# someone-in-somewhere/multimodal_rag

Measured on AMD Instinct MI355X. Metric: chunks embedded/sec + queries/sec top_k=5 over 1M×768 at 1/2/4/8 GPUs, higher is better.
Workload: dtype f16

## Files before the change

multimodal_rag_amd/csrc/search.hip:

```cpp
#include "slab_ring.h"

#include <stdlib.h>

using namespace mmrag;

namespace mmrag_impl {

template <int DT, int WN, int K, int NSTAGE, int NW, bool SEEDED>
__global__ __launch_bounds__(64 * NW, NW / 4) void cosine_topk_kernel(const KParams p) {
#if defined(__HIP_DEVICE_COMPILE__)
#include "slab_ring_body.inc"
#endif
}

template <int K>
struct FullList {
    float v[K];
    long long r[K];
    __device__ inline void init() {
#pragma unroll
        for (int i = 0; i < K; ++i) {
            v[i] = NEG_INF;
            r[i] = LLONG_MAX;
        }
// ... 193 lines not shown
    else launch_main<DT, 8, 0, 2, 16>(p, grid, s);
}

int deep_filter_launch(int dtype, int WN, const KParams &p, int grid_x, int grid_y, hipStream_t s) {
    if (dtype == MMRAG_F8E4M3) return f8_filter_launch(WN, p, grid_x, grid_y, s);
    const dim3 grid(grid_x, grid_y);
    if (dtype == MMRAG_F32) launch_filter<MMRAG_F32>(WN, p, grid, s);
    else if (dtype == MMRAG_F16) launch_filter<MMRAG_F16>(WN, p, grid, s);
    else launch_filter<MMRAG_BF16>(WN, p, grid, s);
    MMRAG_CHECK_HIP(hipGetLastError());
    return MMRAG_OK;
}

template <typename RowT>
int launch_merge(int K, const float *cs, const RowT *cr, long long n_cand, long long inner,
                 long long outer_stride, long long q_stride, int B, int k_out, long long row_offset,
                 float *out_s, long long *out_r, hipStream_t s, float *thr0 = nullptr, float *seed_s = nullptr,
                 int *seed_r = nullptr, long long seed_q_stride = 0) {
    if (K == 5)
        merge_topk_kernel<5, RowT><<<B, 256, 0, s>>>(cs, cr, n_cand, inner, outer_stride, q_stride, k_out,
                                                     row_offset, out_s, out_r, thr0, seed_s, seed_r, seed_q_stride);
    else if (K == 10)
        merge_topk_kernel<10, RowT><<<B, 256, 0, s>>>(cs, cr, n_cand, inner, outer_stride, q_stride, k_out,
                                                      row_offset, out_s, out_r, thr0, seed_s, seed_r, seed_q_stride);
    else
        merge_topk_kernel<20, RowT><<<B, 256, 0, s>>>(cs, cr, n_cand, inner, outer_stride, q_stride, k_out,
                                                      row_offset, out_s, out_r, thr0, seed_s, seed_r, seed_q_stride);
    return MMRAG_OK;
}

__global__ void fill_empty_kernel(float *s, long long *r, long long total) {
    const long long i = (long long)blockIdx.x * blockDim.x + threadIdx.x;
    if (i < total) {
        s[i] = NEG_INF;
        r[i] = -1;
    }
}

__global__ void fill_seed_empty_kernel(float *s, int *r, long long q_stride, int K, long long n_queries) {
    const long long q = (long long)blockIdx.x * blockDim.x + threadIdx.x;
    if (q < n_queries)
        for (int i = 0; i < K; ++i) {
            s[q * q_stride + i] = NEG_INF;
            r[q * q_stride + i] = INT_MAX;
        }
}

}
using namespace mmrag_impl;

extern "C" {

struct WsLayout {
    size_t entries, off_r, off_thr, off_ts, off_tr, off_cnt, cnt_bytes, off_pub, off_pthr, off_tk, xch_end, total;
};
static WsLayout ws_layout(const Plan &pl) {
    WsLayout w;
    w.entries = (size_t)pl.b_pad * pl.n_lists * pl.K;
    w.off_r = w.entries * sizeof(float);
    w.off_thr = w.off_r + w.entries * sizeof(int);
    w.off_ts = w.off_thr + (size_t)pl.b_pad * sizeof(float);
    w.off_tr = (w.off_ts + (size_t)pl.b_pad * pl.K * sizeof(float) + 15) / 16 * 16;
    w.off_cnt = (w.off_tr + (size_t)pl.b_pad * pl.K * sizeof(long long) + 63) / 64 * 64;
    w.cnt_bytes = 0;
    w.off_pub = w.off_cnt + w.cnt_bytes;
    w.off_pthr = w.off_pub + (pl.qs_room ? (size_t)pl.b_pad * pl.grid_x * sizeof(float) : 0);
    w.off_tk = w.off_pthr + (pl.qs_room ? (size_t)pl.b_pad * sizeof(float) : 0);
    w.xch_end = w.off_tk + (pl.qs_room ? ((size_t)pl.grid_y * sizeof(unsigned) + 63) / 64 * 64 : 0);
    w.total = w.xch_end;
    return w;
}

size_t mmrag_cosine_topk_workspace_bytes(int B, int64_t n, int k) {
    if (B <= 0 || n < 0 || k < 1 || k > MMRAG_MAX_K) return 0;
    return ws_layout(make_plan(B, n, k)).total + 256;
}

static int check_search_args(const void *q, const void *corpus, int B, int64_t n, int d, int64_t ld, int dtype,
                             int k) {
    MMRAG_CHECK_ARG(dtype >= 0 && dtype <= MMRAG_F8E4M3, "cosine_topk: bad dtype %d", dtype);
    MMRAG_CHECK_ARG(B > 0, "cosine_topk: B must be positive (got %d)", B);
    MMRAG_CHECK_ARG(k >= 1 && k <= MMRAG_MAX_K, "cosine_topk: k=%d outside 1..%d", k, MMRAG_MAX_K);
    MMRAG_CHECK_ARG(n >= 0 && n < (int64_t)INT_MAX - TM, "cosine_topk: n=%lld out of range", (long long)n);
    MMRAG_CHECK_ARG(d > 0 && ld >= d, "cosine_topk: need 0 < d <= ld (d=%d ld=%lld)", d, (long long)ld);
    const int64_t row_bytes = ld * esize(dtype);
    MMRAG_CHECK_ARG(row_bytes % SLAB == 0,
                    "cosine_topk: row bytes %lld not a multiple of %d (use mmrag_padded_dim)", (long long)row_bytes, SLAB);
    MMRAG_CHECK_ARG(row_bytes * TM < (int64_t)UINT_MAX, "cosine_topk: rows too long");
    MMRAG_CHECK_ARG(q, "cosine_topk: null q");
    MMRAG_CHECK_ARG(n == 0 || corpus, "cosine_topk: null corpus");
    MMRAG_CHECK_ARG(((uintptr_t)q % 16) == 0 && ((uintptr_t)corpus % 16) == 0,
                    "cosine_topk: q/corpus must be 16-byte aligned");
    return MMRAG_OK;
}

int mmrag_internal_cosine_topk_lists_ex(const void *q, const void *corpus, int B, int64_t n, int d, int64_t ld,
                                        int dtype, int k, const uint32_t *alive_bits, void *workspace,
                                        size_t workspace_bytes, void *stream, unsigned dbg) {
    if (int st = check_search_args(q, corpus, B, n, d, ld, dtype, k)) return st;
    if (n == 0) return MMRAG_OK;
    const Plan pl = make_plan(B, n, k, dbg);
    const WsLayout wl = ws_layout(pl);
    if (!workspace || workspace_bytes < wl.total) {
        set_error("cosine_topk: workspace %zu bytes < required %zu", workspace_bytes, wl.total);
        return MMRAG_EWORKSPACE;
    }
    MMRAG_CHECK_ARG(((uintptr_t)workspace % 16) == 0, "cosine_topk: workspace must be 16-byte aligned");

    KParams p;
    p.q = (const char *)q;
    p.corpus = (const char *)corpus;
    p.alive_bits = alive_bits;
    p.cand_s = (float *)workspace;
    p.cand_r = (int *)((char *)workspace + wl.off_r);
    p.n = n;
    p.B = B;
    p.row_bytes = (unsigned)(ld * esize(dtype));
    p.n_tiles = pl.n_tiles;
    p.n_lists = pl.n_lists;
    p.tile0 = 0;
    p.thr0 = nullptr;
    p.dbg = dbg;
    p.stamps = ((dbg & DBG_QS_CLOCK) && workspace_bytes >= wl.total + 256 * (size_t)(pl.grid_x * pl.grid_y)) ? (unsigned long long *)((char *)workspace + wl.total) : nullptr;
    p.walkers = pl.grid_x;
    p.share_l2 = pl.grid_y > 1;
    p.sample_best = nullptr;
    p.pub_best = nullptr;
    p.pub_thr = nullptr;
    p.tickets = nullptr;
    p.p_static = INT_MAX / 2;
    hipStream_t s = (hipStream_t)stream;
    const size_t seed_off = (size_t)(pl.n_lists - 1) * pl.K;
    const int walk_mfma = (dbg & DBG_MFMA32) ? 32 : ((dbg & DBG_MFMA16) ? 16 : (pl.K == 5 ? QSW_DEFAULT_MFMA : 32));
    if (pl.qs_ok && !(dbg & DBG_OLD_QS) && qsw_supported(dtype, p.row_bytes, pl.K, walk_mfma)) {
        const int tiles = (int)((n + QS_TILE_ROWS - 1) / QS_TILE_ROWS);
        const int per = tiles / pl.grid_x;
        p.n_tiles = tiles;
        p.pub_best = nullptr;
        p.pub_thr = nullptr;
        p.tickets = nullptr;
        p.p_static = INT_MAX / 2;
        const bool seed = per >= 12 && !(dbg & DBG_NO_SEED);
        const bool dyn = pl.grid_y == 1 && per >= 24 && !(dbg & DBG_NO_DYN);
        if (seed || dyn) {
            MMRAG_CHECK_HIP(hipMemsetD32Async((hipDeviceptr_t)((char *)workspace + wl.off_pub), (int)TICKET0,
                                              (wl.xch_end - wl.off_pub) / 4, s));
            if (seed) {
                p.pub_best = (float *)((char *)workspace + wl.off_pub);
                p.pub_thr = (float *)((char *)workspace + wl.off_pthr);
            }
            if (dyn) {
                p.tickets = (unsigned *)((char *)workspace + wl.off_tk);
                const int tail = per / 10 > 3 ? per / 10 : 3;
                p.p_static = per - tail;
            }
        }
        if (int st = qsw_launch(dtype, pl.K, walk_mfma, p, pl.grid_x, pl.grid_y, s)) return st;
        MMRAG_CHECK_HIP(hipGetLastError());
        return MMRAG_OK;
    }
    if (pl.qs_ok && qs_supported(dtype, p.row_bytes, pl.K)) {
        const int tiles = (int)((n + QS_TILE_ROWS - 1) / QS_TILE_ROWS);
        float *thr0 = nullptr;
        if (pl.pre_tiles > 0) {
            KParams ks = p;
            ks.n_tiles = pl.pre_tiles * (TM / QS_TILE_ROWS);
            ks.sample_best = (float *)((char *)workspace + wl.off_pub);
            if (int st = qs_launch(dtype, pl.K, ks, pl.grid_x, pl.grid_y, s)) return st;
            thr0 = (float *)((char *)workspace + wl.off_thr);
            if (int st = qs_seed_thresholds(pl.K, ks.sample_best, pl.grid_x, pl.b_pad, thr0, s)) return st;
        }
        p.n_tiles = tiles;
        p.thr0 = thr0;
        if (int st = qs_launch(dtype, pl.K, p, pl.grid_x, pl.grid_y, s)) return st;
        MMRAG_CHECK_HIP(hipGetLastError());
        return MMRAG_OK;
    }
    auto run = [&](int tile0, int n_tiles, int grid_x, const float *thr0) -> int {
        KParams kp = p;
        kp.tile0 = tile0;
        kp.n_tiles = n_tiles;
        kp.thr0 = thr0;
        Plan lp = pl;
        lp.grid_x = grid_x;
        if (dtype == MMRAG_F8E4M3) return f8_lists_launch(lp.K, lp.WN, kp, lp.grid_x, lp.grid_y, s);
        if (dtype == MMRAG_F32) return dispatch_main<MMRAG_F32>(lp, kp, s);
        if (dtype == MMRAG_F16) return dispatch_main<MMRAG_F16>(lp, kp, s);
        return dispatch_main<MMRAG_BF16>(lp, kp, s);
    };
    if (pl.pre_tiles > 0) {
        float *thr0 = (float *)((char *)workspace + wl.off_thr);
        float *top_s = (float *)((char *)workspace + wl.off_ts);
        long long *top_r = (long long *)((char *)workspace + wl.off_tr);
        const int pre = pl.pre_tiles;
        const int pre_grid = pre < pl.grid_x ? pre : pl.grid_x;
        if (int st = run(0, pre, pre_grid, nullptr)) return st;
        MMRAG_CHECK_HIP(hipGetLastError());
        const long long n_cand = (long long)pre_grid * pl.K;
        launch_merge<int>(pl.K, p.cand_s, p.cand_r, n_cand, n_cand, 0, (long long)pl.n_lists * pl.K, B, pl.K, 0, top_s,
                          top_r, s, thr0, p.cand_s + seed_off, p.cand_r + seed_off, (long long)pl.n_lists * pl.K);
        MMRAG_CHECK_HIP(hipGetLastError());
        if (int st = run(pre, pl.n_tiles - pre, pl.grid_x, thr0)) return st;
    } else {
// ... 73 lines not shown
```

multimodal_rag_amd/csrc/search_qsw.hip:

```cpp
#include "search_shared.h"

#include <type_traits>
#include <utility>

using namespace mmrag;

namespace mmrag_impl {

namespace {

template <int DT>
struct WFrag;
template <>
struct WFrag<MMRAG_F16> {
    using T = half8_t;
};
template <>
struct WFrag<MMRAG_BF16> {
    using T = bf16x8_t;
};

template <typename F, int... I>
__device__ __forceinline__ void static_for_impl(F &&f, std::integer_sequence<int, I...>) {
    (f(std::integral_constant<int, I>{}), ...);
}
template <int N, typename F>
__device__ __forceinline__ void static_for(F &&f) {
    static_for_impl(f, std::make_integer_sequence<int, N>{});
}

constexpr int QSW_XCH = 2048 + 64;
constexpr int qsw_lists_bytes(int K, int MS) { return K * (MS == 32 ? 2 : 4) * QS_QROWS * 8; }

struct WRing {
    int G;
    int NST;
};
constexpr WRing qsw_ring(int NK, int K, int MS) {
#if defined(MMRAG_QSW_RING16)
    if (MS == 16 && NK % (MMRAG_QSW_RING16 / 10) == 0) return WRing{MMRAG_QSW_RING16 / 10, MMRAG_QSW_RING16 % 10};
#endif
    const int budget = 160 * 1024 - qsw_lists_bytes(K, MS) - QSW_XCH;
    for (int need = 4; need >= 3; --need)
        for (int g = 4; g >= 1; --g) {
            if (NK % g) continue;
            int nst = budget / (g * QS_TILE_ROWS * SLAB);
            if (nst > 6) nst = 6;
            if (nst >= need) return WRing{g, nst};
        }
    return WRing{1, 2};
}

#define MMRAG_QSW_S32(MNEMONIC, QC, C00, C01, C10, C11, ACC)                                                  \
    asm volatile("v_xad_u32 %[t], %[lo], %[xc], %[st]\n\t"                                                    \
                 "ds_read_b128 %[n0], %[t] offset:%[o0]\n\t"                                                  \
                 "ds_read_b128 %[n1], %[t] offset:%[o1]\n\t" MNEMONIC " %[c00], %[a0], %[q0], " C00 "\n\t"    \
                 MNEMONIC " %[c01], %[a0], %[q1], " C01 "\n\t" MNEMONIC " %[c10], %[a1], %[q0], " C10 "\n\t"  \
                 MNEMONIC " %[c11], %[a1], %[q1], " C11 "\n\t"                                                \
                 "s_waitcnt lgkmcnt(0)"                                                                       \
                 : [c00] ACC(c00), [c01] ACC(c01), [c10] ACC(c10), [c11] ACC(c11), [n0] "=&v"(n0),            \
                   [n1] "=&v"(n1), [t] "=&v"(tmp)                                                             \
                 : [a0] "v"(a0), [a1] "v"(a1), [q0] QC(q0), [q1] QC(q1), [lo] "v"(lo), [st] "s"(st),          \
                   [xc] "i"(XC), [o0] "i"(OFF0), [o1] "i"(OFF1))

template <int DT, bool QA, bool FIRST, int XC, int OFF0, int OFF1, typename FT>
__device__ __forceinline__ void qsw_stmt32(f32x16_t &c00, f32x16_t &c01, f32x16_t &c10, f32x16_t &c11, const FT a0,
                                           const FT a1, const FT q0, const FT q1, FT &n0, FT &n1, const unsigned lo,
                                           const unsigned st) {
    unsigned tmp;
    if constexpr (FIRST) {
        static_assert(QA, "the first k-step's Q fragments live in the accumulator file");
        if constexpr (DT == MMRAG_F16) MMRAG_QSW_S32("v_mfma_f32_32x32x16_f16", "a", "0", "0", "0", "0", "=&v");
        else MMRAG_QSW_S32("v_mfma_f32_32x32x16_bf16", "a", "0", "0", "0", "0", "=&v");
    } else if constexpr (DT == MMRAG_F16) {
        if constexpr (QA) MMRAG_QSW_S32("v_mfma_f32_32x32x16_f16", "a", "%[c00]", "%[c01]", "%[c10]", "%[c11]", "+v");
        else MMRAG_QSW_S32("v_mfma_f32_32x32x16_f16", "v", "%[c00]", "%[c01]", "%[c10]", "%[c11]", "+v");
    } else {
        if constexpr (QA) MMRAG_QSW_S32("v_mfma_f32_32x32x16_bf16", "a", "%[c00]", "%[c01]", "%[c10]", "%[c11]", "+v");
        else MMRAG_QSW_S32("v_mfma_f32_32x32x16_bf16", "v", "%[c00]", "%[c01]", "%[c10]", "%[c11]", "+v");
    }
}

#define MMRAG_QSW_S16(MNEMONIC, QC, D0, D1, D2, D3, D4, D5, D6, D7, ACC)                                      \
    asm volatile(MNEMONIC " %[d0], %[a0], %[q0], " D0 "\n\t"                                                  \
                 "ds_read_b128 %[n0], %[ad] offset:%[o0]\n\t" MNEMONIC " %[d1], %[a0], %[q1], " D1 "\n\t"     \
                 "ds_read_b128 %[n1], %[ad] offset:%[o1]\n\t" MNEMONIC " %[d2], %[a0], %[q2], " D2 "\n\t"     \
                 MNEMONIC " %[d3], %[a0], %[q3], " D3 "\n\t" MNEMONIC " %[d4], %[a1], %[q0], " D4 "\n\t"      \
                 MNEMONIC " %[d5], %[a1], %[q1], " D5 "\n\t" MNEMONIC " %[d6], %[a1], %[q2], " D6 "\n\t"      \
                 MNEMONIC " %[d7], %[a1], %[q3], " D7 "\n\t"                                                  \
                 "s_waitcnt lgkmcnt(0)"                                                                       \
                 : [d0] ACC(d0), [d1] ACC(d1), [d2] ACC(d2), [d3] ACC(d3), [d4] ACC(d4), [d5] ACC(d5),        \
                   [d6] ACC(d6), [d7] ACC(d7), [n0] "=&v"(n0), [n1] "=&v"(n1)                                 \
                 : [a0] "v"(a0), [a1] "v"(a1), [q0] QC(q0), [q1] QC(q1), [q2] QC(q2), [q3] QC(q3),            \
                   [ad] "v"(adr), [o0] "i"(OFF0), [o1] "i"(OFF1))
#define MMRAG_QSW_S16_ACC(MNEMONIC, QC)                                                                       \
// ... 16 lines not shown
        if constexpr (QA) MMRAG_QSW_S16_ACC("v_mfma_f32_16x16x32_bf16", "a");
        else MMRAG_QSW_S16_ACC("v_mfma_f32_16x16x32_bf16", "v");
    }
}

__device__ __forceinline__ void qsw_stage_addr(unsigned &a_lo, unsigned &a_hi, const unsigned lo, const unsigned st) {
    asm volatile("v_add_u32 %0, %2, %3\n\tv_xad_u32 %1, %2, 64, %3" : "=&v"(a_lo), "=&v"(a_hi) : "v"(lo), "s"(st));
}

__device__ __forceinline__ float max16_raw(float x0, float x1, float x2, float x3, float x4, float x5, float x6, float x7,
                                           float x8, float x9, float x10, float x11, float x12, float x13, float x14,
                                           float x15) {
    float r;
    asm("v_max3_f32 %0, %1, %2, %3\n\t"
        "v_max3_f32 %0, %0, %4, %5\n\t"
        "v_max3_f32 %0, %0, %6, %7\n\t"
        "v_max3_f32 %0, %0, %8, %9\n\t"
        "v_max3_f32 %0, %0, %10, %11\n\t"
        "v_max3_f32 %0, %0, %12, %13\n\t"
        "v_max3_f32 %0, %0, %14, %15\n\t"
        "v_max_f32 %0, %0, %16"
        : "=&v"(r)
        : "v"(x0), "v"(x1), "v"(x2), "v"(x3), "v"(x4), "v"(x5), "v"(x6), "v"(x7), "v"(x8), "v"(x9), "v"(x10), "v"(x11),
          "v"(x12), "v"(x13), "v"(x14), "v"(x15));
    return r;
}

constexpr int CP_SC1 = 16;

}

template <int DT, int NK, int K, int MS, bool NT>
__global__ __launch_bounds__(256, 1) void cosine_topk_walk_kernel(const KParams p) {
#if defined(__HIP_DEVICE_COMPILE__)
    using FT = typename WFrag<DT>::T;
    static_assert(MS == 32 || MS == 16, "MFMA shape");
    constexpr int R = QS_TILE_ROWS;
    static_assert(R == 64, "statements are written for 64-row tiles");
    constexpr int RB = R / 32;
    constexpr int SLABB = R * SLAB;
    constexpr int NQB = MS == 32 ? 2 : 4;
    constexpr int QW = MS;
    constexpr int NSUB = 64 / QW;
    constexpr int NGRP = 16 / NSUB;
    constexpr WRing RING = qsw_ring(NK, K, MS);
    constexpr int G = RING.G, NST = RING.NST;
    constexpr int SPT = NK / G;
    constexpr int STAGE = G * SLABB;
    constexpr int PPS = G * RB;
    constexpr int KSTG = G * 4;
    constexpr int KST = MS == 32 ? NK * 4 : NK * 2;
    constexpr int QA_STEPS = 64 / NQB;
    constexpr int LISTS = qsw_lists_bytes(K, MS);
    constexpr int LOOK = (NST + 1 + SPT - 1) / SPT + 1;
    static_assert(NST >= 3 && NST * STAGE + LISTS + QSW_XCH <= 160 * 1024, "LDS");
    static_assert((NST - 1) * PPS <= 56, "vmcnt range");
    static_assert((G - 1) * SLABB + 48 * SLAB + 2048 < 65536, "ds_read immediate offset");
    static_assert(2 * PPS == KSTG, "one piece after every other statement");
    constexpr int LANDT = ((NST - 2) * PPS + 1 + SPT * PPS - 1) / (SPT * PPS);
    static_assert(LANDT >= 1 && LANDT * SPT * PPS - 1 >= (NST - 2) * PPS, "exchange pieces land before they are used");
    static_assert(LOOK <= 6, "ticket slots");

    __shared__ __attribute__((aligned(1024))) char smem[NST * STAGE + LISTS + QSW_XCH];
    float *lists = (float *)(smem + NST * STAGE);
    float *const gather_lds = (float *)(smem + NST * STAGE + LISTS);
    float *const poll_lds = (float *)(smem + NST * STAGE + LISTS + 1024);
    int *const tk_lds = (int *)(smem + NST * STAGE + LISTS + 2048);

    const int tid = threadIdx.x;
    const int lane = tid & 63;
    const int wave = __builtin_amdgcn_readfirstlane(tid >> 6);
    const int ql = lane & (QW - 1);
    const int sub = lane / QW;
    auto dev_dbg = [&](unsigned flag) -> bool {
#if defined(MMRAG_QSW_DEV)
        return (p.dbg & flag) != 0;
#else
        (void)flag;
        return false;
#endif
    };
    const unsigned long long t_entry = (p.dbg & DBG_QS_CLOCK) ? __builtin_amdgcn_s_memrealtime() : 0ull;

    const unsigned RBy = p.row_bytes;
    const int walkers = p.walkers;
    const int bx = (int)blockIdx.x % walkers;
    const int by = (int)blockIdx.x / walkers;
    const int q0 = by * QS_QROWS;
    const int p_static = p.p_static;
    auto pos_tile = [&](int pos) -> int {
        if (pos < p_static) return bx + pos * walkers;
        return p_static * walkers + (int)((unsigned)__builtin_amdgcn_readfirstlane(tk_lds[pos & 7]) - TICKET0);
    };

    unsigned c_off0;
    {
        const int row = (wave * RB) * 8 + (lane >> 3);
        c_off0 = (unsigned)row * RBy + (unsigned)(((lane & 7) ^ ((row >> 1) & 7)) * 16);
    }
    auto c_off = [&](int i) -> unsigned { return i == 0 ? c_off0 : (c_off0 ^ 64u) + 8u * RBy; };
    int is_pos = 0;
    int fill_tile = bx;
    __amdgpu_buffer_rsrc_t fill_rsrc;
    typedef __attribute__((address_space(3))) char *lds_char_t;
    const lds_char_t wave_lds = (lds_char_t)(lds_ptr_t)(smem + wave * (RB * 1024));
    lds_char_t stage_lds = wave_lds;
    auto fill_open = [&]() {
        const bool real = (unsigned)fill_tile < (unsigned)p.n_tiles && !dev_dbg(DBG_QS_NO_DMA);
        const long long row0 = real ? (dev_dbg(DBG_QS_DMA_L2) ? (long long)bx * R : (long long)fill_tile * R) : 0;
        const long long rows_left = p.n - row0;
        const unsigned c_bytes = real ? (unsigned)((rows_left < R ? rows_left : (long long)R) * (long long)RBy) : 0u;
        fill_rsrc = __builtin_amdgcn_make_buffer_rsrc((void *)(p.corpus + (size_t)row0 * RBy), 0, c_bytes, 0x00020000);
    };
    auto next_fill = [&](auto is_sg_c, int buf) {
        constexpr int IS_SG = decltype(is_sg_c)::value;
        if constexpr (IS_SG == 0) {
            if (is_pos != 0) fill_tile = pos_tile(is_pos);
            fill_open();
            ++is_pos;
        }
        stage_lds = wave_lds + buf * STAGE;
        asm volatile("" : "+s"(stage_lds));
    };
    unsigned koff = 0;
    auto issue_piece = [&](auto is_sg_c, auto pi_c) {
        constexpr int IS_SG = decltype(is_sg_c)::value, PI = decltype(pi_c)::value;
        constexpr int g = PI / RB, i = PI % RB;
        if constexpr (i == 0) asm volatile("s_movk_i32 %0, %1" : "=s"(koff) : "n"((IS_SG * G + g) * SLAB));
        __builtin_amdgcn_raw_ptr_buffer_load_lds(fill_rsrc, (lds_ptr_t)(stage_lds + g * SLABB + i * 1024), 16, c_off(i),
                                                 koff, 0, NT ? 2 : 0);
    };

    const bool any_tile = bx < p.n_tiles;
    if (any_tile)
        static_for<NST>([&](auto st_c) {
            constexpr int st = decltype(st_c)::value;
            next_fill(std::integral_constant<int, st % SPT>{}, st);
            static_for<PPS>([&](auto pi_c) { issue_piece(std::integral_constant<int, st % SPT>{}, pi_c); });
        });
    asm volatile("s_movk_i32 %0, %1" : "=s"(koff) : "n"(((NST - 1) % SPT) * G * SLAB));

    FT qf[NQB][KST];
    float thr[NQB];
    static_for<NQB>([&](auto qb_c) {
        constexpr int qb = decltype(qb_c)::value;
        const int qrow = q0 + wave * 64 + qb * QW + ql;
        const bool live = qrow < p.B;
        const char *src = p.q + (size_t)(live ? qrow : 0) * RBy + sub * 16;
#pragma unroll
        for (int s = 0; s < KST; ++s) {
            FT v = *(const FT *)(src + s * (16 * NSUB));
            if (!live) v = FT{};
            qf[qb][s] = v;
        }
        thr[qb] = !live ? INFINITY : NEG_INF;
    });
    float *const my_lists = lists + tid;
    auto lst_v = [&](int qb, int i) -> float & { return my_lists[(qb * 2 * K + i) * QS_QROWS]; };
    auto lst_r = [&](int qb, int i) -> int & { return *(int *)&my_lists[(qb * 2 * K + K + i) * QS_QROWS]; };
#pragma unroll
    for (int qb = 0; qb < NQB; ++qb)
#pragma unroll
        for (int i = 0; i < K; ++i) {
            lst_v(qb, i) = NEG_INF;
            lst_r(qb, i) = INT_MAX;
        }

    const int sw = (ql >> 1) & 7;
    const unsigned lane_off0 = (unsigned)(ql * SLAB + ((sub ^ sw) * 16));
    const unsigned lane_off64 = lane_off0 ^ 64u;
    const unsigned smem_base = (unsigned)(size_t)(lds_ptr_t)smem;

    auto lane_now = []() -> int {
        int l;
        asm volatile("v_mbcnt_lo_u32_b32 %0, -1, 0\n\tv_mbcnt_hi_u32_b32 %0, -1, %0" : "=v"(l));
        return l;
    };
    f32x16_t c32[MS == 32 ? 4 : 1];
    f32x4_t c16[MS == 16 ? 16 : 1];
    auto score = [&](auto qb_c, auto gi_c, int i) -> float {
        constexpr int qb = decltype(qb_c)::value, gi = decltype(gi_c)::value;
        if constexpr (MS == 32) return c32[(gi >> 2) * 2 + qb][4 * (gi & 3) + i];
        else return c16[gi * 4 + qb][i];
    };
    auto grp_row = [](int gi) -> int { return MS == 32 ? (gi >> 2) * 32 + 8 * (gi & 3) : gi * 16; };
    auto strike = [&](unsigned m0, unsigned m1, const int sub) {
        static_for<NQB>([&](auto qb_c) {
            static_for<NGRP>([&](auto gi_c) {
                constexpr int qb = decltype(qb_c)::value, gi = decltype(gi_c)::value;
                constexpr int r0 = MS == 32 ? (gi >> 2) * 32 + 8 * (gi & 3) : gi * 16;
                const unsigned m = (r0 < 32 ? m0 : m1) >> ((r0 & 31) + 4 * sub);
#pragma unroll
                for (int i = 0; i < 4; ++i) {
                    const bool ok = (m >> i) & 1u;
                    if constexpr (MS == 32) {
                        constexpr int a = (gi >> 2) * 2 + qb, e = 4 * (gi & 3);
                        c32[a][e + i] = ok ? c32[a][e + i] : NEG_INF;
                    } else {
                        c16[gi * 4 + qb][i] = ok ? c16[gi * 4 + qb][i] : NEG_INF;
                    }
                }
            });
        });
    };

    auto select = [&](auto qb_c, const int row_base, float *const my_lists) {
        auto lst_v = [&](int qb, int i) -> float & { return my_lists[(qb * 2 * K + i) * QS_QROWS]; };
        auto lst_r = [&](int qb, int i) -> int & { return *(int *)&my_lists[(qb * 2 * K + K + i) * QS_QROWS]; };
// ... 45 lines not shown
        constexpr int DENSE_AT = NE == 16 ? 8 : 12;
        if (__builtin_amdgcn_ballot_w64(__builtin_popcount(mask) > DENSE_AT) == 0ull) {
            while (__builtin_amdgcn_ballot_w64(mask != 0u) != 0ull) {
                const bool valid = mask != 0u;
                const unsigned e = (unsigned)__builtin_ctz(mask | (1u << (NE - 1)));
                mask &= mask - 1u;
                float lvl[NE];
                static_for<NE>([&](auto e_c) {
                    constexpr int x = decltype(e_c)::value;
                    lvl[x] = score(qb_c, std::integral_constant<int, x / 4>{}, x % 4);
                });
#pragma unroll
                for (int w = NE / 2, b = 0; w >= 1; w >>= 1, ++b) {
                    const bool bit = (e >> b) & 1u;
#pragma unroll
                    for (int i = 0; i < w; ++i) lvl[i] = bit ? lvl[2 * i + 1] : lvl[2 * i];
                }
                const float sc = lvl[0];
                const int row = MS == 32 ? (int)(((e >> 4) << 5) + (((e >> 2) & 3u) << 3) + (e & 3u))
                                         : (int)(((e >> 2) << 4) + (e & 3u));
                L.insert_strict_flat(valid && sc >= t ? sc : NEG_INF, row_base + row);
                t = fmaxf(t, L.v[K - 1]);
            }
        } else {
            static_for<NGRP>([&](auto gi_c) {
                constexpr int gi = decltype(gi_c)::value;
                const float a0 = score(qb_c, gi_c, 0), a1 = score(qb_c, gi_c, 1);
                const float a2 = score(qb_c, gi_c, 2), a3 = score(qb_c, gi_c, 3);
                if (__builtin_amdgcn_ballot_w64(fmaxf(fmaxf(a0, a1), fmaxf(a2, a3)) >= t) != 0ull) {
#pragma clang loop unroll(disable)
                    for (int i = 0; i < 4; ++i) {
                        const float s = i == 0 ? a0 : (i == 1 ? a1 : (i == 2 ? a2 : a3));
                        const bool pass = s >= t;
                        if (__builtin_amdgcn_ballot_w64(pass) != 0ull) {
                            L.insert_strict(pass ? s : NEG_INF, row_base + grp_row(gi) + i);
                            t = fmaxf(t, L.v[K - 1]);
                        }
                    }
                }
            });
        }
        float u = fmaxf(L.v[K - 1], __shfl_xor(L.v[K - 1], QW));
#pragma unroll
        for (int i = 0; i + 1 < K; ++i) u = fmaxf(u, fminf(L.v[i], __shfl_xor(L.v[K - 2 - i], QW)));
        if constexpr (NSUB == 4) u = fmaxf(u, __shfl_xor(u, 32));
        thr[qb] = fmaxf(t, u);
#pragma unroll
        for (int i = 0; i < K; ++i) {
            lst_v(qb, i) = L.v[i];
            lst_r(qb, i) = L.r[i];
        }
    };

    const bool seeding = p.pub_best != nullptr;
    const int n_resp = (QS_QROWS + walkers - 1) / walkers;
    auto publish_bests = [&](const int ql, const int sub, float *const my_lists) {
        auto lst_v = [&](int qb, int i) -> float & { return my_lists[(qb * 2 * K + i) * QS_QROWS]; };
        float *dst = p.pub_best + ((size_t)by * walkers + bx) * QS_QROWS + wave * 64 + ql;
        static_for<NQB>([&](auto qb_c) {
            constexpr int qb = decltype(qb_c)::value;
            float v = lst_v(qb, 0);
            v = fmaxf(v, __shfl_xor(v, QW));
            if constexpr (NSUB == 4) v = fmaxf(v, __shfl_xor(v, 32));
            if (sub == 0) __hip_atomic_store(dst + qb * QW, v, __ATOMIC_RELAXED, __HIP_MEMORY_SCOPE_AGENT);
        });
    };
    auto gather_issue = [&](int q) {
        const int ln = lane_now();
        const __amdgpu_buffer_rsrc_t rs = __builtin_amdgcn_make_buffer_rsrc(
            (void *)(p.pub_best + (size_t)by * walkers * QS_QROWS), 0, (unsigned)(walkers * QS_QROWS * 4), 0x00020000);
#pragma unroll
        for (int c = 0; c < 4; ++c)
            __builtin_amdgcn_raw_ptr_buffer_load_lds(rs, (lds_ptr_t)((char *)gather_lds + c * 256), 4,
                                                     (unsigned)(((c * 64 + ln) * QS_QROWS + q) * 4), 0, 0, CP_SC1);
    };
    auto compute_thr = [&](int q) {
        const int ln = lane_now();
        float v[4];
#pragma unroll
        for (int c = 0; c < 4; ++c) v[c] = (c * 64 + ln) < walkers ? gather_lds[c * 64 + ln] : NEG_INF;
        const float t = wave_kth_largest<K>(v[0], v[1], v[2], v[3], ln);
        if (ln == 0)
            __hip_atomic_store(p.pub_thr + (size_t)by * QS_QROWS + q, t, __ATOMIC_RELAXED, __HIP_MEMORY_SCOPE_AGENT);
    };
    auto poll_issue = [&]() {
        const __amdgpu_buffer_rsrc_t rs = __builtin_amdgcn_make_buffer_rsrc(
            (void *)(p.pub_thr + (size_t)by * QS_QROWS), 0, QS_QROWS * 4, 0x00020000);
        __builtin_amdgcn_raw_ptr_buffer_load_lds(rs, (lds_ptr_t)poll_lds, 16, (unsigned)(lane_now() * 16), 0, 0, CP_SC1);
    };
    auto poll_consume = [&](const int ql) {
        static_for<NQB>([&](auto qb_c) {
            constexpr int qb = decltype(qb_c)::value;
            thr[qb] = fmaxf(thr[qb], poll_lds[wave * 64 + qb * QW + ql]);
        });
    };
    constexpr int STEP = LANDT;
    const int span = n_resp * STEP + LANDT + 1;
    const int pub1 = span + 1 > 5 ? span + 1 : 5;
    auto polled_at = [&](int t) -> bool { return t >= 1 + LANDT && (t < pub1 + span + 4 || (t & 3) == 3); };
    const int quiet = pub1 + span + 4 + LANDT;

    unsigned long long t0c = 0, t0r = 0;
    if (p.dbg & DBG_QS_CLOCK) {
        t0c = __builtin_amdgcn_s_memtime();
        t0r = __builtin_amdgcn_s_memrealtime();
    }
    if (any_tile) {
        FT fa0, fa1, fb0, fb1;
        wait_vmcnt<(NST - 1) * PPS>();
        __builtin_amdgcn_s_barrier();
        {
            const char *st = smem + lane_off0;
            fa0 = *(const FT *)(st);
            fa1 = *(const FT *)(st + (MS == 32 ? 32 * SLAB : 16 * SLAB));
        }
        int cur_tile = bx;
        for (int ti = 0; (unsigned)cur_tile < (unsigned)p.n_tiles; ++ti) {
            unsigned adr_lo = 0, adr_hi = 0;
            if constexpr (MS == 16)
                qsw_stage_addr(adr_lo, adr_hi, lane_off0, smem_base + (unsigned)(((ti * SPT) % NST) * STAGE));
            unsigned tkv;
            const bool want_ticket = ti + LOOK >= p_static && wave == 0;
            if (want_ticket) {
                unsigned long long saved_exec;
                asm volatile("s_mov_b64 %1, exec\n\t"
                             "s_mov_b64 exec, 1\n\t"
                             "global_atomic_add %0, %2, %3, %4 sc0\n\t"
                             "s_mov_b64 exec, %1"
                             : "=&v"(tkv), "=&s"(saved_exec)
                             : "v"(0u), "v"(1u), "s"(p.tickets + by)
                             : "memory");
            }
            static_for<SPT>([&](auto sg_c) {
                constexpr int sg = decltype(sg_c)::value;
                const int it = ti * SPT + sg;
                const unsigned st_cur = smem_base + (unsigned)((it % NST) * STAGE);
                const unsigned st_nxt = smem_base + (unsigned)(((it + 1) % NST) * STAGE);
                static_for<KSTG>([&](auto j_c) {
                    constexpr int j = decltype(j_c)::value;
                    constexpr int g = j / 4, m = j % 4;
                    constexpr bool last = j == KSTG - 1;
                    constexpr int nj = last ? 0 : j + 1;
                    constexpr int ng = nj / 4, nm = nj % 4;
                    constexpr int slab = sg * G + g;
                    const unsigned st = last ? st_nxt : st_cur;
                    FT &x0 = (j & 1) ? fb0 : fa0, &x1 = (j & 1) ? fb1 : fa1;
                    FT &y0 = (j & 1) ? fa0 : fb0, &y1 = (j & 1) ? fa1 : fb1;
                    if constexpr (MS == 32) {
                        constexpr int ks = slab * 4 + m;
                        qsw_stmt32<DT, (ks < QA_STEPS), ks == 0, (nm & 1) * 32, ng * SLABB, ng * SLABB + 32 * SLAB, FT>(
                            c32[0], c32[1], c32[2], c32[3], x0, x1, qf[0][ks], qf[1][ks], y0, y1,
                            (nm & 2) ? lane_off64 : lane_off0, st);
                    } else {
                        constexpr int ks = slab * 2 + (m >> 1), rp = m & 1;
                        constexpr int o0 = ng * SLABB + (nm & 1) * (32 * SLAB);
                        if constexpr (last) qsw_stage_addr(adr_lo, adr_hi, lane_off0, st_nxt);
                        qsw_stmt16<DT, (ks < QA_STEPS), ks == 0, o0, o0 + 16 * SLAB, FT>(
                            c16[rp * 8 + 0], c16[rp * 8 + 1], c16[rp * 8 + 2], c16[rp * 8 + 3], c16[rp * 8 + 4],
                            c16[rp * 8 + 5], c16[rp * 8 + 6], c16[rp * 8 + 7], x0, x1, qf[0][ks], qf[1][ks], qf[2][ks],
                            qf[3][ks], y0, y1, (nm >> 1) ? adr_hi : adr_lo);
                    }
                    if constexpr (j == KSTG - 2) {
                        wait_vmcnt<(NST - 2) * PPS>();
                        if (!dev_dbg(DBG_QS_NO_BARRIER)) __builtin_amdgcn_s_barrier();
                        next_fill(std::integral_constant<int, (NST + sg) % SPT>{}, it % NST);
                    }
                    if constexpr (j == KSTG - 1)
                        issue_piece(std::integral_constant<int, (NST + sg) % SPT>{}, std::integral_constant<int, 0>{});
                    else if constexpr ((j & 1) == 1)
                        issue_piece(std::integral_constant<int, (NST + sg + SPT - 1) % SPT>{},
                                    std::integral_constant<int, (j + 1) / 2>{});
                });
            });
            asm volatile("s_nop 15\n\ts_nop 7");
            const long long row0 = (long long)cur_tile * R;
            if (row0 + R > p.n || p.alive_bits != nullptr) {
                const long long left = p.n - row0;
                unsigned m0 = left >= 32 ? 0xffffffffu : ((1u << (int)left) - 1u);
                unsigned m1 = left >= 64 ? 0xffffffffu : (left > 32 ? ((1u << (int)(left - 32)) - 1u) : 0u);
                if (p.alive_bits != nullptr) {
                    typedef const __attribute__((address_space(4))) uint32_t *scalar_words_t;
                    const scalar_words_t words = (scalar_words_t)p.alive_bits;
                    m0 &= words[row0 >> 5];
                    if (left > 32) m1 &= words[(row0 >> 5) + 1];
                }
                strike(m0, m1, lane_now() / QW);
            }
            const int ln = lane_now();
            const int ql_t = ln & (QW - 1), sub_t = ln / QW;
            float *const lists_t = lists + wave * 64 + ln;
            const int row_base = (int)row0 + 4 * sub_t;
            if (!(p.dbg & DBG_QS_NO_SELECT)) {
                static_for<NQB>([&](auto qb_c) { select(qb_c, row_base, lists_t); });
            } else {
                if constexpr (MS == 32) asm volatile("" ::"v"(c32[0]), "v"(c32[1]), "v"(c32[2]), "v"(c32[3]));
                else {
#pragma unroll
                    for (int e = 0; e < 16; ++e) asm volatile("" ::"v"(c16[e]));
                }
            }
            if (seeding && ti >= quiet) {
                if (((ti - LANDT) & 3) == 3) poll_consume(ql_t);
                if ((ti & 3) == 3 && wave == 0) poll_issue();
            } else if (seeding) {
                if (ti >= LANDT && polled_at(ti - LANDT)) poll_consume(ql_t);
                if (ti == 0 || ti == pub1) publish_bests(ql_t, sub_t, lists_t);
                if (wave == 0) {
                    const int rel = ti > pub1 ? ti - (pub1 + 1) : ti - 1;
                    const int jc = rel - LANDT, jg = rel;
                    if (jc >= 0 && jc % STEP == 0 && jc / STEP < n_resp && bx + (jc / STEP) * walkers < QS_QROWS)
                        compute_thr(bx + (jc / STEP) * walkers);
                    if (jg >= 0 && jg % STEP == 0 && jg / STEP < n_resp && bx + (jg / STEP) * walkers < QS_QROWS)
                        gather_issue(bx + (jg / STEP) * walkers);
                    if (polled_at(ti)) poll_issue();
                }
            }
            if ((p.dbg & DBG_QS_CLOCK) && p.stamps != nullptr && ti < 28 && wave == 0 && ln == 0)
                p.stamps[32 * blockIdx.x + 4 + ti] = __builtin_amdgcn_s_memrealtime();
            if (want_ticket) {
                wait_vmcnt<SPT * PPS>();
                unsigned long long saved_exec;
                const unsigned slot = (unsigned)(size_t)(lds_ptr_t)(tk_lds + ((ti + LOOK) & 7));
                asm volatile("s_mov_b64 %0, exec\n\t"
                             "s_mov_b64 exec, 1\n\t"
                             "ds_write_b32 %1, %2\n\t"
                             "s_mov_b64 exec, %0"
                             : "=&s"(saved_exec)
                             : "v"(slot), "v"(tkv)
                             : "memory");
            }
            cur_tile = pos_tile(ti + 1);
        }
    }
    const int tid_e = wave * 64 + lane_now();
    if ((p.dbg & DBG_QS_CLOCK) && p.stamps != nullptr && tid_e == 0) {
        p.stamps[32 * blockIdx.x] = __builtin_amdgcn_s_memtime() - t0c;
        p.stamps[32 * blockIdx.x + 1] = __builtin_amdgcn_s_memrealtime() - t0r;
        p.stamps[32 * blockIdx.x + 2] = t0r - t_entry;
        p.stamps[32 * blockIdx.x + 3] = t_entry;
    }
    __syncthreads();
    if (q0 + tid_e < p.B) {
        const int w = tid_e >> 6, qb = (tid_e / QW) & (NQB - 1), c = tid_e & (QW - 1);
        const float *la = lists + w * 64 + c + (qb * 2 * K) * QS_QROWS;
        TopList<K> m;
#pragma unroll
        for (int i = 0; i < K; ++i) {
            m.v[i] = la[i * QS_QROWS];
            m.r[i] = __float_as_int(la[(K + i) * QS_QROWS]);
        }
        for (int s = 1; s < NSUB; ++s) {
            const float *lb = la + s * QW;
            for (int i = 0; i < K; ++i) {
                const float x = lb[i * QS_QROWS];
                const int xr = __float_as_int(lb[(K + i) * QS_QROWS]);
                if (xr == INT_MAX || !better(x, xr, m.v[K - 1], m.r[K - 1])) break;
                m.insert_ordered(x, xr);
            }
        }
        const size_t base = ((size_t)(q0 + tid_e) * p.n_lists + bx) * K;
#pragma unroll
        for (int i = 0; i < K; ++i) {
            p.cand_s[base + i] = m.v[i];
            p.cand_r[base + i] = m.r[i];
        }
        if (bx == 0 && p.n_lists > walkers) {
            const size_t seed = ((size_t)(q0 + tid_e) * p.n_lists + (p.n_lists - 1)) * K;
#pragma unroll
            for (int i = 0; i < K; ++i) {
                p.cand_s[seed + i] = NEG_INF;
                p.cand_r[seed + i] = INT_MAX;
            }
        }
    }
#endif
}

bool qsw_supported(int dtype, unsigned row_bytes, int K, int mfma) {
    if (dtype != MMRAG_F16 && dtype != MMRAG_BF16) return false;
    if (K != 5) return false;
    const unsigned nk = row_bytes / SLAB;
#if defined(MMRAG_QSW_DEV)
// ... 46 lines not shown
```

multimodal_rag_amd/csrc/search_shared.h:

```cpp
#pragma once
#include "mmrag_internal.h"
#include "tile_dma.h"

#include <limits.h>

namespace mmrag_impl {

constexpr float NEG_INF = -__builtin_inff();

__device__ inline bool better(float s, long long r, float s2, long long r2) {
    return s > s2 || (s == s2 && r < r2);
}

template <int K>
struct TopList {
    float v[K];
    int r[K];
    __device__ inline void init() {
#pragma unroll
        for (int i = 0; i < K; ++i) {
            v[i] = NEG_INF;
            r[i] = INT_MAX;
        }
    }
// ... 7 lines not shown
            const int nxr = b ? r[j] : xr;
            v[j] = nv;
            x = nx;
            r[j] = nr;
            xr = nxr;
        }
    }
    __device__ inline void insert_strict(float x, int xr) {
#pragma unroll
        for (int j = 0; j < K; ++j) {
            const bool b = x > v[j];
            const float nv = b ? x : v[j];
            const float nx = b ? v[j] : x;
            const int nr = b ? xr : r[j];
            const int nxr = b ? r[j] : xr;
            v[j] = nv;
            x = nx;
            r[j] = nr;
            xr = nxr;
        }
    }
    __device__ inline void insert_strict_flat(float x, int xr) {
        bool c[K];
#pragma unroll
        for (int j = 0; j < K; ++j) c[j] = x > v[j];
#pragma unroll
        for (int j = K - 1; j >= 1; --j) {
            v[j] = c[j] ? (c[j - 1] ? v[j - 1] : x) : v[j];
            r[j] = c[j] ? (c[j - 1] ? r[j - 1] : xr) : r[j];
        }
        v[0] = c[0] ? x : v[0];
        r[0] = c[0] ? xr : r[0];
    }
};

struct KParams {
    const char *q;
    const char *corpus;
    const uint32_t *alive_bits;
    float *cand_s;
    int *cand_r;
    long long n;
    int B;
    unsigned row_bytes;
    int n_tiles;
    int n_lists;
    int tile0;
    int walkers;
    int share_l2;
    const float *thr0;
    unsigned dbg;
    unsigned long long *stamps;
    float *sample_best;
    float *pub_best;
    float *pub_thr;
    unsigned *tickets;
    int p_static;
    int tile_stride;
    unsigned *deep_cnt;
    int deep_cap;
};
constexpr unsigned TICKET0 = 0xff800000u;

constexpr unsigned DBG_QS_NO_SELECT = 16u, DBG_QS_NO_DMA = 32u, DBG_QS_NO_BARRIER = 64u, DBG_QS_DMA_L2 = 512u, DBG_QS_NO_WAIT = 1024u;
constexpr unsigned DBG_QS_CLOCK = 256u;

template <int K>
__device__ inline float wave_kth_largest(float a, float b, float c, float d, int lane) {
    auto ce = [](float &x, float &y) {
        const float hi = fmaxf(x, y), lo = fminf(x, y);
        x = hi;
        y = lo;
    };
    ce(a, b);
    ce(c, d);
    ce(a, c);
    ce(b, d);
    ce(b, c);
    float res = NEG_INF;
    for (int r = 0; r < K; ++r) {
        float m = a;
#pragma unroll
        for (int off = 32; off >= 1; off >>= 1) m = fmaxf(m, __shfl_xor(m, off));
        res = m;
        const unsigned long long owners = __builtin_amdgcn_ballot_w64(a == m);
        if (owners != 0ull && lane == (int)__builtin_ctzll(owners)) {
            a = b;
            b = c;
            c = d;
            d = NEG_INF;
        }
    }
    return res;
}

bool qs_supported(int dtype, unsigned row_bytes, int K);
constexpr int QS_TILE_ROWS = 64;
constexpr int QS_QROWS = 256;
int qs_launch(int dtype, int K, const KParams &p, int grid_x, int grid_y, hipStream_t s);
int qs_seed_thresholds(int K, const float *best, int walkers, int n_queries, float *thr0, hipStream_t s);

constexpr int QSW_DEFAULT_MFMA = 16;
bool qsw_supported(int dtype, unsigned row_bytes, int K, int mfma);
int qsw_launch(int dtype, int K, int mfma, const KParams &p, int grid_x, int grid_y, hipStream_t s);

int deep_filter_launch(int dtype, int WN, const KParams &p, int grid_x, int grid_y, hipStream_t s);

int f8_lists_launch(int K, int WN, const KParams &p, int grid_x, int grid_y, hipStream_t s);
int f8_filter_launch(int WN, const KParams &p, int grid_x, int grid_y, hipStream_t s);


}
```

Before: 662,900.

## Replace gather-based threshold seeding with atomic max over K walker classes

Workgroups previously published per-walker bests, then had designated waves gather every walker's best and compute a k-th-largest threshold to publish for polling. Now each walker atomically maxes an order-preserving key into one of K class slots (bx mod K), and pollers take the min over the K class maxima as a lower bound on the k-th best. This removes the gather/compute_thr stages and their schedule, and publishes repeatedly (first NPUB tiles, then every fourth) so the bound tightens early. Polls now fetch K buffers into a resized LDS exchange area, and seeding is disabled when grid_x is smaller than the class count or the workspace lacks room.

```diff
diff --git a/multimodal_rag_amd/csrc/search.hip b/multimodal_rag_amd/csrc/search.hip
--- a/multimodal_rag_amd/csrc/search.hip
+++ b/multimodal_rag_amd/csrc/search.hip
@@ -269,7 +269,7 @@
 extern "C" {
 
 struct WsLayout {
-    size_t entries, off_r, off_thr, off_ts, off_tr, off_cnt, cnt_bytes, off_pub, off_pthr, off_tk, xch_end, total;
+    size_t entries, off_r, off_thr, off_ts, off_tr, off_cnt, cnt_bytes, off_pub, off_pthr, off_tk, off_gmax, xch_end, total;
 };
 static WsLayout ws_layout(const Plan &pl) {
     WsLayout w;
@@ -284,6 +284,8 @@
     w.off_pthr = w.off_pub + (pl.qs_room ? (size_t)pl.b_pad * pl.grid_x * sizeof(float) : 0);
     w.off_tk = w.off_pthr + (pl.qs_room ? (size_t)pl.b_pad * sizeof(float) : 0);
     w.xch_end = w.off_tk + (pl.qs_room ? ((size_t)pl.grid_y * sizeof(unsigned) + 63) / 64 * 64 : 0);
+    const size_t gmax_bytes = (size_t)pl.grid_y * QSW_CLASSES * QS_QROWS * sizeof(unsigned);
+    w.off_gmax = pl.qs_room && w.off_tk - w.off_pub >= gmax_bytes ? w.off_tk - gmax_bytes : 0;
     w.total = w.xch_end;
     return w;
 }
@@ -342,8 +344,8 @@
     p.walkers = pl.grid_x;
     p.share_l2 = pl.grid_y > 1;
     p.sample_best = nullptr;
-    p.pub_best = nullptr;
-    p.pub_thr = nullptr;
+    p.grp_max = nullptr;
+    p.reserved0 = nullptr;
     p.tickets = nullptr;
     p.p_static = INT_MAX / 2;
     hipStream_t s = (hipStream_t)stream;
@@ -353,19 +355,15 @@
         const int tiles = (int)((n + QS_TILE_ROWS - 1) / QS_TILE_ROWS);
         const int per = tiles / pl.grid_x;
         p.n_tiles = tiles;
-        p.pub_best = nullptr;
-        p.pub_thr = nullptr;
+        p.grp_max = nullptr;
         p.tickets = nullptr;
         p.p_static = INT_MAX / 2;
-        const bool seed = per >= 12 && !(dbg & DBG_NO_SEED);
+        const bool seed = per >= 12 && pl.grid_x >= QSW_CLASSES && wl.off_gmax != 0 && !(dbg & DBG_NO_SEED);
         const bool dyn = pl.grid_y == 1 && per >= 24 && !(dbg & DBG_NO_DYN);
         if (seed || dyn) {
-            MMRAG_CHECK_HIP(hipMemsetD32Async((hipDeviceptr_t)((char *)workspace + wl.off_pub), (int)TICKET0,
-                                              (wl.xch_end - wl.off_pub) / 4, s));
-            if (seed) {
-                p.pub_best = (float *)((char *)workspace + wl.off_pub);
-                p.pub_thr = (float *)((char *)workspace + wl.off_pthr);
-            }
+            const size_t fill0 = seed ? wl.off_gmax : wl.off_tk;
+            MMRAG_CHECK_HIP(hipMemsetAsync((char *)workspace + fill0, 0, wl.xch_end - fill0, s));
+            if (seed) p.grp_max = (unsigned *)((char *)workspace + wl.off_gmax);
             if (dyn) {
                 p.tickets = (unsigned *)((char *)workspace + wl.off_tk);
                 const int tail = per / 10 > 3 ? per / 10 : 3;
diff --git a/multimodal_rag_amd/csrc/search_qsw.hip b/multimodal_rag_amd/csrc/search_qsw.hip
--- a/multimodal_rag_amd/csrc/search_qsw.hip
+++ b/multimodal_rag_amd/csrc/search_qsw.hip
@@ -29,7 +29,7 @@
     static_for_impl(f, std::make_integer_sequence<int, N>{});
 }
 
-constexpr int QSW_XCH = 2048 + 64;
+constexpr int qsw_xch_bytes(int K) { return K * 1024 + 64; }
 constexpr int qsw_lists_bytes(int K, int MS) { return K * (MS == 32 ? 2 : 4) * QS_QROWS * 8; }
 
 struct WRing {
@@ -40,7 +40,7 @@
 #if defined(MMRAG_QSW_RING16)
     if (MS == 16 && NK % (MMRAG_QSW_RING16 / 10) == 0) return WRing{MMRAG_QSW_RING16 / 10, MMRAG_QSW_RING16 % 10};
 #endif
-    const int budget = 160 * 1024 - qsw_lists_bytes(K, MS) - QSW_XCH;
+    const int budget = 160 * 1024 - qsw_lists_bytes(K, MS) - qsw_xch_bytes(K);
     for (int need = 4; need >= 3; --need)
         for (int g = 4; g >= 1; --g) {
             if (NK % g) continue;
@@ -163,6 +163,12 @@
     constexpr int KST = MS == 32 ? NK * 4 : NK * 2;
     constexpr int QA_STEPS = 64 / NQB;
     constexpr int LISTS = qsw_lists_bytes(K, MS);
+    constexpr int QSW_XCH = qsw_xch_bytes(K);
+#if !defined(MMRAG_QSW_RING16)
+    static_assert(MS != 16 || K != 5 || NK != 12 || (G == 3 && NST == 4), "768-d ring: 4 stages of 24 KiB");
+    static_assert(MS != 16 || K != 5 || NK != 8 || (G == 2 && NST == 6), "512-d ring: 6 stages of 16 KiB");
+    static_assert(MS != 16 || K != 5 || NK != 6 || (G == 3 && NST == 4), "384-d ring: 4 stages of 24 KiB");
+#endif
     constexpr int LOOK = (NST + 1 + SPT - 1) / SPT + 1;
     static_assert(NST >= 3 && NST * STAGE + LISTS + QSW_XCH <= 160 * 1024, "LDS");
     static_assert((NST - 1) * PPS <= 56, "vmcnt range");
@@ -174,9 +180,8 @@
 
     __shared__ __attribute__((aligned(1024))) char smem[NST * STAGE + LISTS + QSW_XCH];
     float *lists = (float *)(smem + NST * STAGE);
-    float *const gather_lds = (float *)(smem + NST * STAGE + LISTS);
-    float *const poll_lds = (float *)(smem + NST * STAGE + LISTS + 1024);
-    int *const tk_lds = (int *)(smem + NST * STAGE + LISTS + 2048);
+    unsigned *const poll_lds = (unsigned *)(smem + NST * STAGE + LISTS);
+    int *const tk_lds = (int *)(smem + NST * STAGE + LISTS + K * 1024);
 
     const int tid = threadIdx.x;
     const int lane = tid & 63;
@@ -265,6 +270,7 @@
             qf[qb][s] = v;
         }
         thr[qb] = !live ? INFINITY : NEG_INF;
+        if constexpr (qb == NQB / 2 - 1) __builtin_amdgcn_sched_barrier(0);
     });
     float *const my_lists = lists + tid;
     auto lst_v = [&](int qb, int i) -> float & { return my_lists[(qb * 2 * K + i) * QS_QROWS]; };
@@ -416,53 +422,44 @@
         }
     };
 
-    const bool seeding = p.pub_best != nullptr;
-    const int n_resp = (QS_QROWS + walkers - 1) / walkers;
-    auto publish_bests = [&](const int ql, const int sub, float *const my_lists) {
+    const bool seeding = p.grp_max != nullptr;
+    static_assert(K * 1024 + 8 * (int)sizeof(int) <= QSW_XCH, "poll buffer: K pieces of 1 KiB, then the ticket slots");
+    auto publish_max = [&](const int ql, const int sub, float *const my_lists) {
         auto lst_v = [&](int qb, int i) -> float & { return my_lists[(qb * 2 * K + i) * QS_QROWS]; };
-        float *dst = p.pub_best + ((size_t)by * walkers + bx) * QS_QROWS + wave * 64 + ql;
+        unsigned *dst = p.grp_max + ((size_t)by * K + (unsigned)bx % (unsigned)K) * QS_QROWS + wave * 64 + ql;
         static_for<NQB>([&](auto qb_c) {
             constexpr int qb = decltype(qb_c)::value;
             float v = lst_v(qb, 0);
             v = fmaxf(v, __shfl_xor(v, QW));
             if constexpr (NSUB == 4) v = fmaxf(v, __shfl_xor(v, 32));
-            if (sub == 0) __hip_atomic_store(dst + qb * QW, v, __ATOMIC_RELAXED, __HIP_MEMORY_SCOPE_AGENT);
+            const unsigned bits = __float_as_uint(v);
+            const unsigned key = bits ^ ((unsigned)((int)bits >> 31) | 0x80000000u);
+            if (sub == 0) (void)__hip_atomic_fetch_max(dst + qb * QW, key, __ATOMIC_RELAXED, __HIP_MEMORY_SCOPE_AGENT);
         });
-    };
-    auto gather_issue = [&](int q) {
-        const int ln = lane_now();
-        const __amdgpu_buffer_rsrc_t rs = __builtin_amdgcn_make_buffer_rsrc(
-            (void *)(p.pub_best + (size_t)by * walkers * QS_QROWS), 0, (unsigned)(walkers * QS_QROWS * 4), 0x00020000);
-#pragma unroll
-        for (int c = 0; c < 4; ++c)
-            __builtin_amdgcn_raw_ptr_buffer_load_lds(rs, (lds_ptr_t)((char *)gather_lds + c * 256), 4,
-                                                     (unsigned)(((c * 64 + ln) * QS_QROWS + q) * 4), 0, 0, CP_SC1);
-    };
-    auto compute_thr = [&](int q) {
-        const int ln = lane_now();
-        float v[4];
-#pragma unroll
-        for (int c = 0; c < 4; ++c) v[c] = (c * 64 + ln) < walkers ? gather_lds[c * 64 + ln] : NEG_INF;
-        const float t = wave_kth_largest<K>(v[0], v[1], v[2], v[3], ln);
-        if (ln == 0)
-            __hip_atomic_store(p.pub_thr + (size_t)by * QS_QROWS + q, t, __ATOMIC_RELAXED, __HIP_MEMORY_SCOPE_AGENT);
     };
     auto poll_issue = [&]() {
         const __amdgpu_buffer_rsrc_t rs = __builtin_amdgcn_make_buffer_rsrc(
-            (void *)(p.pub_thr + (size_t)by * QS_QROWS), 0, QS_QROWS * 4, 0x00020000);
-        __builtin_amdgcn_raw_ptr_buffer_load_lds(rs, (lds_ptr_t)poll_lds, 16, (unsigned)(lane_now() * 16), 0, 0, CP_SC1);
+            (void *)(p.grp_max + (size_t)by * K * QS_QROWS), 0, K * QS_QROWS * 4, 0x00020000);
+        const unsigned off = (unsigned)(lane_now() * 16);
+#pragma unroll
+        for (int g = 0; g < K; ++g)
+            __builtin_amdgcn_raw_ptr_buffer_load_lds(rs, (lds_ptr_t)((char *)poll_lds + g * 1024), 16, off, g * 1024, 0,
+                                                     CP_SC1);
     };
     auto poll_consume = [&](const int ql) {
         static_for<NQB>([&](auto qb_c) {
             constexpr int qb = decltype(qb_c)::value;
-            thr[qb] = fmaxf(thr[qb], poll_lds[wave * 64 + qb * QW + ql]);
+            const unsigned *src = poll_lds + wave * 64 + qb * QW + ql;
+            unsigned key = src[0];
+#pragma unroll
+            for (int g = 1; g < K; ++g) key = min(key, src[g * QS_QROWS]);
+            const float bound = __uint_as_float(key ^ (~(unsigned)((int)key >> 31) | 0x80000000u));
+            thr[qb] = fmaxf(thr[qb], key == 0u ? NEG_INF : bound);
         });
     };
-    constexpr int STEP = LANDT;
-    const int span = n_resp * STEP + LANDT + 1;
-    const int pub1 = span + 1 > 5 ? span + 1 : 5;
-    auto polled_at = [&](int t) -> bool { return t >= 1 + LANDT && (t < pub1 + span + 4 || (t & 3) == 3); };
-    const int quiet = pub1 + span + 4 + LANDT;
+    constexpr int NPUB = 8;
+    constexpr int POLLS = NPUB + 2;
+    auto polled_at = [&](int t) -> bool { return t >= 1 && (t < POLLS || (t & 3) == 3); };
 
     unsigned long long t0c = 0, t0r = 0;
     if (p.dbg & DBG_QS_CLOCK) {
@@ -563,22 +560,7 @@
                     for (int e = 0; e < 16; ++e) asm volatile("" ::"v"(c16[e]));
                 }
             }
-            if (seeding && ti >= quiet) {
-                if (((ti - LANDT) & 3) == 3) poll_consume(ql_t);
-                if ((ti & 3) == 3 && wave == 0) poll_issue();
-            } else if (seeding) {
-                if (ti >= LANDT && polled_at(ti - LANDT)) poll_consume(ql_t);
-                if (ti == 0 || ti == pub1) publish_bests(ql_t, sub_t, lists_t);
-                if (wave == 0) {
-                    const int rel = ti > pub1 ? ti - (pub1 + 1) : ti - 1;
-                    const int jc = rel - LANDT, jg = rel;
-                    if (jc >= 0 && jc % STEP == 0 && jc / STEP < n_resp && bx + (jc / STEP) * walkers < QS_QROWS)
-                        compute_thr(bx + (jc / STEP) * walkers);
-                    if (jg >= 0 && jg % STEP == 0 && jg / STEP < n_resp && bx + (jg / STEP) * walkers < QS_QROWS)
-                        gather_issue(bx + (jg / STEP) * walkers);
-                    if (polled_at(ti)) poll_issue();
-                }
-            }
+            if (seeding && ti >= LANDT && polled_at(ti - LANDT)) poll_consume(ql_t);
             if ((p.dbg & DBG_QS_CLOCK) && p.stamps != nullptr && ti < 28 && wave == 0 && ln == 0)
                 p.stamps[32 * blockIdx.x + 4 + ti] = __builtin_amdgcn_s_memrealtime();
             if (want_ticket) {
@@ -592,6 +574,10 @@
                              : "=&s"(saved_exec)
                              : "v"(slot), "v"(tkv)
                              : "memory");
+            }
+            if (seeding) {
+                if (ti < NPUB || (ti & 3) == 1) publish_max(ql_t, sub_t, lists_t);
+                if (wave == 0 && polled_at(ti)) poll_issue();
             }
             cur_tile = pos_tile(ti + 1);
         }
diff --git a/multimodal_rag_amd/csrc/search_shared.h b/multimodal_rag_amd/csrc/search_shared.h
--- a/multimodal_rag_amd/csrc/search_shared.h
+++ b/multimodal_rag_amd/csrc/search_shared.h
@@ -83,15 +83,15 @@
     unsigned dbg;
     unsigned long long *stamps;
     float *sample_best;
-    float *pub_best;
-    float *pub_thr;
+    unsigned *grp_max;
+    float *reserved0;
     unsigned *tickets;
     int p_static;
     int tile_stride;
     unsigned *deep_cnt;
     int deep_cap;
 };
-constexpr unsigned TICKET0 = 0xff800000u;
+constexpr unsigned TICKET0 = 0u;
 
 constexpr unsigned DBG_QS_NO_SELECT = 16u, DBG_QS_NO_DMA = 32u, DBG_QS_NO_BARRIER = 64u, DBG_QS_DMA_L2 = 512u, DBG_QS_NO_WAIT = 1024u;
 constexpr unsigned DBG_QS_CLOCK = 256u;
@@ -131,6 +131,7 @@
 int qs_launch(int dtype, int K, const KParams &p, int grid_x, int grid_y, hipStream_t s);
 int qs_seed_thresholds(int K, const float *best, int walkers, int n_queries, float *thr0, hipStream_t s);
 
+constexpr int QSW_CLASSES = 5;
 constexpr int QSW_DEFAULT_MFMA = 16;
 bool qsw_supported(int dtype, unsigned row_bytes, int K, int mfma);
 int qsw_launch(int dtype, int K, int mfma, const KParams &p, int grid_x, int grid_y, hipStream_t s);
```

Measured after the change: 612,500. -7.6%, worse.
